# RuyiLian/CheckerPose

Measured on AMD Instinct MI355X. Metric: crops/sec forward (256x256, npt=512), higher is better.
Workload: dtype bf16; 1 GPU; LMO 'ape' hr18GNN2_res6_gnn3Skip_mlpQuery npt=512, PoseNet_GNNskip forward, deterministic random-init weights; global_batch=256, parallelism=dp1 (no forward collective), launch=hipGraph replay of 104 kernel launches

## Files before the change

checkerpose_amd/csrc/common.h:

```cpp
#pragma once
#include <hip/hip_runtime.h>
#include <stdint.h>
#include <atomic>

#include "../../include/checkerpose_hip.h"

typedef __attribute__((ext_vector_type(4))) float f32x4;
typedef __attribute__((ext_vector_type(4))) uint32_t u32x4;
typedef __attribute__((ext_vector_type(2))) uint32_t u32x2;
typedef __attribute__((ext_vector_type(8))) __bf16 bf16x8;

__device__ __forceinline__ float bf16_bits_to_f32(uint32_t h) { return __uint_as_float(h << 16); }
__device__ __forceinline__ uint32_t f32_to_bf16_bits(float f) {
  __bf16 b = (__bf16)f;
  return (uint32_t)__builtin_bit_cast(uint16_t, b);
}
typedef __bf16 cp_bf16x2 __attribute__((ext_vector_type(2)));
typedef float cp_f32x2 __attribute__((ext_vector_type(2)));
__device__ __forceinline__ uint32_t pack_bf16x2(float lo, float hi) {
  return __builtin_bit_cast(uint32_t, __builtin_convertvector(cp_f32x2{lo, hi}, cp_bf16x2));
}

__device__ __forceinline__ float cp_act_slope(int act, float slope) { return act == 1 ? 0.f : (act == 2 ? slope : 1.f); }
__device__ __forceinline__ float cp_act_apply(float v, float s) { return fmaxf(v, fmaf(v, s, 0.f)); }

__device__ __forceinline__ __amdgpu_buffer_rsrc_t cp_dma_rsrc(const void* base) {
  return __builtin_amdgcn_make_buffer_rsrc(const_cast<void*>(base), 0, 0x7fffffff, 0x00020000);
}
__device__ __forceinline__ void cp_lds_dma16(__amdgpu_buffer_rsrc_t rs, uint32_t off, void* lds_dst) {
  __builtin_amdgcn_raw_ptr_buffer_load_lds(rs, (__attribute__((address_space(3))) void*)lds_dst, 16, off, 0, 0, 0);
}

typedef short cp_s16x2 __attribute__((ext_vector_type(2)));
__device__ __forceinline__ uint32_t relu_bf16x2(uint32_t v) {
  return __builtin_bit_cast(uint32_t, __builtin_elementwise_max(__builtin_bit_cast(cp_s16x2, v), cp_s16x2{0, 0}));
}

typedef _Float16 cp_h2 __attribute__((ext_vector_type(2)));
__device__ __forceinline__ uint32_t pack_f16x2_sat(float a, float b) {
  cp_h2 r;
  r.x = (_Float16)__builtin_amdgcn_fmed3f(a, -65504.f, 65504.f);
  r.y = (_Float16)__builtin_amdgcn_fmed3f(b, -65504.f, 65504.f);
  return __builtin_bit_cast(uint32_t, r);
}
__device__ __forceinline__ uint32_t pkmax3_f16(uint32_t a, uint32_t b, uint32_t c) {
  return __builtin_bit_cast(uint32_t, __builtin_elementwise_maximum(__builtin_bit_cast(cp_h2, a),
                            __builtin_elementwise_maximum(__builtin_bit_cast(cp_h2, b), __builtin_bit_cast(cp_h2, c))));
}
__device__ __forceinline__ void pkmax5x4_f16(uint32_t* m, const u32x4& a, const u32x4& b, const u32x4& c, const u32x4& d) {
  asm("v_pk_maximum3_f16 %0, %0, %4, %8\n\t"
      "v_pk_maximum3_f16 %1, %1, %5, %9\n\t"
      "v_pk_maximum3_f16 %2, %2, %6, %10\n\t"
      "v_pk_maximum3_f16 %3, %3, %7, %11\n\t"
      "v_pk_maximum3_f16 %0, %0, %12, %16\n\t"
      "v_pk_maximum3_f16 %1, %1, %13, %17\n\t"
      "v_pk_maximum3_f16 %2, %2, %14, %18\n\t"
      "v_pk_maximum3_f16 %3, %3, %15, %19"
      : "+v"(m[0]), "+v"(m[1]), "+v"(m[2]), "+v"(m[3])
      : "v"(a.x), "v"(a.y), "v"(a.z), "v"(a.w), "v"(b.x), "v"(b.y), "v"(b.z), "v"(b.w),
        "v"(c.x), "v"(c.y), "v"(c.z), "v"(c.w), "v"(d.x), "v"(d.y), "v"(d.z), "v"(d.w));
}
__device__ __forceinline__ float f16_lo(uint32_t w) { return (float)__builtin_bit_cast(cp_h2, w).x; }
__device__ __forceinline__ float f16_hi(uint32_t w) { return (float)__builtin_bit_cast(cp_h2, w).y; }
constexpr uint32_t CP_F16X2_NEG_INF = 0xFC00FC00u;

typedef _Float16 f16x8 __attribute__((ext_vector_type(8)));
template <bool H>
__device__ __forceinline__ f32x4 cp_mma16(const u32x4& w, const u32x4& a, const f32x4& acc) {
  if constexpr (H) return __builtin_amdgcn_mfma_f32_16x16x32_f16(__builtin_bit_cast(f16x8, w), __builtin_bit_cast(f16x8, a), acc, 0, 0, 0);
  else return __builtin_amdgcn_mfma_f32_16x16x32_bf16(__builtin_bit_cast(bf16x8, w), __builtin_bit_cast(bf16x8, a), acc, 0, 0, 0);
}
__device__ __forceinline__ void cp_f16_saturate_on() { asm volatile("s_setreg_imm32_b32 hwreg(HW_REG_MODE, 23, 1), 1" ::: "memory"); }
__device__ __forceinline__ uint32_t pack_f16x2_ovfl(float a, float b) {
  cp_h2 r;
  r.x = (_Float16)a;
  r.y = (_Float16)b;
  return __builtin_bit_cast(uint32_t, r);
}
template <bool H>
__device__ __forceinline__ uint32_t cp_pack2(float lo, float hi) {
  if constexpr (H) return pack_f16x2_ovfl(lo, hi);
  else return pack_bf16x2(lo, hi);
}
template <bool H>
__device__ __forceinline__ u32x4 cp_pack8(const float* f) {
  u32x4 v; v.x = cp_pack2<H>(f[0], f[1]); v.y = cp_pack2<H>(f[2], f[3]); v.z = cp_pack2<H>(f[4], f[5]); v.w = cp_pack2<H>(f[6], f[7]);
  return v;
}
__device__ __forceinline__ uint32_t f32_to_f16_bits_sat(float f) {
  return (uint32_t)__builtin_bit_cast(uint16_t, (_Float16)__builtin_amdgcn_fmed3f(f, -65504.f, 65504.f));
}
__device__ __forceinline__ float f16_bits_to_f32(uint32_t h) { return (float)__builtin_bit_cast(_Float16, (uint16_t)h); }
__device__ __forceinline__ uint32_t f32_to_half_bits(float f, int dtype) { return dtype == CP_F16 ? f32_to_f16_bits_sat(f) : f32_to_bf16_bits(f); }

struct F32Tag { using elem = float; static constexpr int E = 4; static constexpr int dtype = CP_F32; };
struct BF16Tag { using elem = uint16_t; static constexpr int E = 8; static constexpr int dtype = CP_BF16; };
struct F16Tag { using elem = uint16_t; static constexpr int E = 8; static constexpr int dtype = CP_F16; };

template <typename Tag> struct Vec16;
template <> struct Vec16<F32Tag> {
  static __device__ __forceinline__ void unpack(const u32x4& v, float* f) {
    f[0] = __uint_as_float(v.x); f[1] = __uint_as_float(v.y); f[2] = __uint_as_float(v.z); f[3] = __uint_as_float(v.w);
  }
  static __device__ __forceinline__ u32x4 pack(const float* f) {
    u32x4 v; v.x = __float_as_uint(f[0]); v.y = __float_as_uint(f[1]); v.z = __float_as_uint(f[2]); v.w = __float_as_uint(f[3]);
    return v;
  }
};
template <> struct Vec16<BF16Tag> {
  static __device__ __forceinline__ void unpack(const u32x4& v, float* f) {
    f[0] = __uint_as_float(v.x << 16); f[1] = __uint_as_float(v.x & 0xffff0000u);
    f[2] = __uint_as_float(v.y << 16); f[3] = __uint_as_float(v.y & 0xffff0000u);
    f[4] = __uint_as_float(v.z << 16); f[5] = __uint_as_float(v.z & 0xffff0000u);
    f[6] = __uint_as_float(v.w << 16); f[7] = __uint_as_float(v.w & 0xffff0000u);
  }
  static __device__ __forceinline__ u32x4 pack(const float* f) {
    u32x4 v; v.x = pack_bf16x2(f[0], f[1]); v.y = pack_bf16x2(f[2], f[3]);
    v.z = pack_bf16x2(f[4], f[5]); v.w = pack_bf16x2(f[6], f[7]);
    return v;
  }
};

template <> struct Vec16<F16Tag> {
  static __device__ __forceinline__ void unpack(const u32x4& v, float* f) {
    f[0] = f16_lo(v.x); f[1] = f16_hi(v.x); f[2] = f16_lo(v.y); f[3] = f16_hi(v.y);
    f[4] = f16_lo(v.z); f[5] = f16_hi(v.z); f[6] = f16_lo(v.w); f[7] = f16_hi(v.w);
  }
  static __device__ __forceinline__ u32x4 pack(const float* f) { return cp_pack8<true>(f); }
};

__device__ __forceinline__ void cp_up_coord(float s, int o, int n, int& i0, int& step, float& l1) {
#pragma clang fp contract(off)
  const float f = s * (float)o;
  i0 = (int)f;
  step = i0 < n - 1 ? 1 : 0;
  l1 = f - (float)i0;
}
__device__ __forceinline__ float cp_one_minus(float l1) {
#pragma clang fp contract(off)
  return 1.f - l1;
}
__device__ __forceinline__ float cp_bilerp(float a, float b, float c, float d, float lx0, float lx1, float ly0, float ly1) {
#pragma clang fp contract(off)
  const float t = __builtin_fmaf(lx1, b, lx0 * a);
  const float u = __builtin_fmaf(lx1, d, lx0 * c);
  return __builtin_fmaf(ly1, u, ly0 * t);
}

template <typename Tag> __device__ __forceinline__ float load_elem(const void* p, size_t i);
template <> __device__ __forceinline__ float load_elem<F32Tag>(const void* p, size_t i) { return ((const float*)p)[i]; }
template <> __device__ __forceinline__ float load_elem<BF16Tag>(const void* p, size_t i) {
  return bf16_bits_to_f32(((const uint16_t*)p)[i]);
}
template <> __device__ __forceinline__ float load_elem<F16Tag>(const void* p, size_t i) { return f16_bits_to_f32(((const uint16_t*)p)[i]); }
template <typename Tag> __device__ __forceinline__ void store_elem(void* p, size_t i, float v);
template <> __device__ __forceinline__ void store_elem<F16Tag>(void* p, size_t i, float v) { ((uint16_t*)p)[i] = (uint16_t)f32_to_f16_bits_sat(v); }
template <> __device__ __forceinline__ void store_elem<F32Tag>(void* p, size_t i, float v) { ((float*)p)[i] = v; }
template <> __device__ __forceinline__ void store_elem<BF16Tag>(void* p, size_t i, float v) {
  ((uint16_t*)p)[i] = (uint16_t)f32_to_bf16_bits(v);
}

#ifdef CP_DEBUG_KNOBS
#include <stdlib.h>
static inline const char* cp_knob(const char* name) { return getenv(name); }
#else
static inline const char* cp_knob(const char*) { return nullptr; }
#endif
extern std::atomic<int> g_cp_deterministic;
static inline bool cp_deterministic() { return g_cp_deterministic.load(std::memory_order_relaxed) != 0; }
uint32_t* cp_status_word(bool create);
void cp_mark_kernel(const char* fmt, ...);
#define CP_LAUNCH(kernel, ...) do { cp_mark_kernel("%s", #kernel); hipLaunchKernelGGL(kernel, __VA_ARGS__); } while (0)
static inline int cp_check_launch() {
  hipError_t e = hipGetLastError();
  return e == hipSuccess ? CP_OK : CP_ERR_HIP;
}
struct CpDeviceOnce {
  std::atomic<unsigned long long> bits[4];
  bool needed(int dev) const { return !((bits[(dev >> 6) & 3].load(std::memory_order_acquire) >> (dev & 63)) & 1ull); }
  void mark(int dev) { bits[(dev >> 6) & 3].fetch_or(1ull << (dev & 63), std::memory_order_release); }
};
static inline int cp_current_device() {
  int dev = 0;
  return hipGetDevice(&dev) == hipSuccess ? dev : -1;
}
#define CP_LDS_ATTR_ONCE(once, dev, ...)                                                     \
  do {                                                                                       \
    if ((dev) < 0) return CP_ERR_HIP;                                                        \
    if ((once).needed(dev)) {                                                                \
      if (!(__VA_ARGS__)) return CP_ERR_HIP;                                                 \
      (once).mark(dev);                                                                      \
    }                                                                                        \
  } while (0)
static inline bool cp_set_max_lds(const void* fn, size_t bytes) {
  return hipFuncSetAttribute(fn, hipFuncAttributeMaxDynamicSharedMemorySize, (int)bytes) == hipSuccess;
}
static inline int cp_num_cus() {
  static std::atomic<int> cache[256];
  const int dev = cp_current_device();
  if (dev < 0) return 0;
  int n = cache[dev & 255].load(std::memory_order_relaxed);
  if (!n) {
    if (hipDeviceGetAttribute(&n, hipDeviceAttributeMultiprocessorCount, dev) != hipSuccess) return 0;
    cache[dev & 255].store(n, std::memory_order_relaxed);
  }
  return n;
}
static inline bool cp_aligned16(const void* p) { return (((uintptr_t)p) & 15u) == 0; }
static inline size_t cp_align16_up(size_t n) { return (n + 15) & ~(size_t)15; }
static inline bool cp_misaligned(const void* q, uintptr_t mask) { return ((uintptr_t)q & mask) != 0; }
static inline bool cp_act_ok(int act, float slope) { return act != 2  || (slope >= 0.f && slope <= 1.f); }
static inline int cp_elem_size(int dtype) { return (dtype == CP_BF16 || dtype == CP_F16) ? 2 : 4; }
```

checkerpose_amd/csrc/conv3x3_halo.hip:

```cpp
#include <stdlib.h>

#include "common.h"
#include <cstring>

struct HaloParams {
  const void* in; const void* w; const float* scale; const float* shift; const void* res; void* out;
  int B, H, W, Cin, in_cs, in_coff, nchunk, Cout, ngroups, NB;
  int tiles_x, tiles_y, total_tiles;
  int act; float slope;
  uint32_t in_bytes, w_bytes;
  long long o_base, o_sb, o_sy, o_sx;
  int Hs, Ws; float up_sy, up_sx;
  const float* seg_w; const float* seg_b; float* seg_out; int seg_S;
};

constexpr int HTH = 8, HTW = 16, HPW = HTW + 2, HPH = HTH + 2, HNPIX = 192;
constexpr int HPLANE = HNPIX * 16, HBUF = 4 * HPLANE;
constexpr int USRH = 7, USRW = 11, USPIX = 80, USBUF = USPIX * 64;

template <typename Tag> struct MmaH;
template <> struct MmaH<F32Tag> {
  static __device__ __forceinline__ void run(const u32x4& w, const u32x4& a, f32x4& acc) {
    acc = __builtin_amdgcn_mfma_f32_16x16x4f32(__uint_as_float(w.x), __uint_as_float(a.x), acc, 0, 0, 0);
    acc = __builtin_amdgcn_mfma_f32_16x16x4f32(__uint_as_float(w.y), __uint_as_float(a.y), acc, 0, 0, 0);
    acc = __builtin_amdgcn_mfma_f32_16x16x4f32(__uint_as_float(w.z), __uint_as_float(a.z), acc, 0, 0, 0);
    acc = __builtin_amdgcn_mfma_f32_16x16x4f32(__uint_as_float(w.w), __uint_as_float(a.w), acc, 0, 0, 0);
  }
};
template <> struct MmaH<BF16Tag> {
  static __device__ __forceinline__ void run(const u32x4& w, const u32x4& a, f32x4& acc) {
    acc = __builtin_amdgcn_mfma_f32_16x16x32_bf16(__builtin_bit_cast(bf16x8, w), __builtin_bit_cast(bf16x8, a), acc, 0, 0, 0);
  }
};

template <typename Tag, bool HAS_RES>
__global__ __launch_bounds__(256) void conv3x3_halo_kernel(const HaloParams p) {
  constexpr int E = Tag::E;
  constexpr int KCH = 4 * E;
  constexpr int ES = 16 / E;
  extern __shared__ __attribute__((aligned(16))) unsigned char smem[];

  const int label = blockIdx.x & 7, slot = blockIdx.x >> 3;
  const int nblk = slot % p.NB;
  const int t = label * ((p.total_tiles + 7) >> 3) + slot / p.NB;
  if (t >= p.total_tiles) return;
  const int tpi = p.tiles_x * p.tiles_y;
  const int b = t / tpi;
  const int trem = t - b * tpi;
  const int ty = trem / p.tiles_x, tx = trem - ty * p.tiles_x;
  const int y0 = ty * HTH, x0 = tx * HTW;

  const int tid = threadIdx.x;
  const int lane = tid & 63;
  const int wave = __builtin_amdgcn_readfirstlane(tid >> 6);
  const int x = lane & 15, q = lane >> 4;
  const int g = nblk * 4 + wave;
  const bool wave_active = g < p.ngroups;

  const __amdgpu_buffer_rsrc_t rsrc = __builtin_amdgcn_make_buffer_rsrc(const_cast<void*>(p.in), 0, p.in_bytes, 0x00020000);
  const __amdgpu_buffer_rsrc_t wrsrc = __builtin_amdgcn_make_buffer_rsrc(const_cast<void*>(p.w), 0, p.w_bytes, 0x00020000);

  uint32_t s_goff[3];
  uint32_t s_lds[3];
  int s_cq[3];
#pragma unroll
  for (int k = 0; k < 3; ++k) {
    const int i = tid + 256 * k;
    const int hp = i >> 2, pq = i & 3;
    const int py = hp / HPW, px = hp - py * HPW;
    const int gy = y0 - 1 + py, gx = x0 - 1 + px;
    const bool ok = (hp < HPH * HPW) & ((unsigned)gy < (unsigned)p.H) & ((unsigned)gx < (unsigned)p.W);
    s_goff[k] = ok ? (uint32_t)(((b * p.H + gy) * p.W + gx) * p.in_cs + p.in_coff + pq * E) : 0xFFFFFFFFu;
    s_lds[k] = (uint32_t)(pq * HPLANE + (hp < HNPIX ? hp : 0) * 16);
    s_cq[k] = pq * E;
  }
  const bool s_do[3] = {true, true, (tid + 512) < HNPIX * 4};

  auto stage_load = [&](u32x4* v, int c) {
    const int c0 = c * KCH;
#pragma unroll
    for (int k = 0; k < 3; ++k) {
      const bool ok = (s_goff[k] != 0xFFFFFFFFu) & (c0 + s_cq[k] < p.Cin);
      const uint32_t off = ok ? (s_goff[k] + (uint32_t)c0) * ES : 0x80000000u;
      v[k] = __builtin_bit_cast(u32x4, __builtin_amdgcn_raw_buffer_load_b128(rsrc, off, 0, 0));
    }
  };
  auto stage_write = [&](const u32x4* v, int buf) {
#pragma unroll
    for (int k = 0; k < 3; ++k)
      if (s_do[k]) *(u32x4*)(smem + buf * HBUF + s_lds[k]) = v[k];
  };

  f32x4 acc[HTH][2];
#pragma unroll
  for (int mt = 0; mt < HTH; ++mt) { acc[mt][0] = f32x4{0.f, 0.f, 0.f, 0.f}; acc[mt][1] = f32x4{0.f, 0.f, 0.f, 0.f}; }

  const uint32_t wbase = ((uint32_t)(wave_active ? g : 0) * p.nchunk * 18u * 64u + lane) * 16u;
  auto w_load = [&](u32x4* w, int c, int tap) {
    const uint32_t off = wbase + ((uint32_t)c * 18u + (uint32_t)tap * 2u) * 1024u;
    w[0] = __builtin_bit_cast(u32x4, __builtin_amdgcn_raw_buffer_load_b128(wrsrc, off, 0, 0));
    w[1] = __builtin_bit_cast(u32x4, __builtin_amdgcn_raw_buffer_load_b128(wrsrc, off + 1024u, 0, 0));
  };
  const uint32_t a_lane = (uint32_t)(q * HPLANE + x * 16);
  auto a_load = [&](u32x4* a, int buf, int tap) {
    const int r = tap / 3, s = tap - 3 * r;
    const unsigned char* base = smem + buf * HBUF + a_lane + (r * HPW + s) * 16;
#pragma unroll
    for (int mt = 0; mt < HTH; ++mt) a[mt] = *(const u32x4*)(base + mt * HPW * 16);
  };
  auto mma = [&](const u32x4* a, const u32x4* w) {
#pragma unroll
    for (int mt = 0; mt < HTH; ++mt) {
      MmaH<Tag>::run(w[0], a[mt], acc[mt][0]);
      MmaH<Tag>::run(w[1], a[mt], acc[mt][1]);
    }
  };

  u32x4 sv[3];
  stage_load(sv, 0);
  u32x4 w0[2], w1[2], w2[2], aA[HTH], aB[HTH];
  w_load(w0, 0, 0);
  w_load(w1, 0, 1);
  stage_write(sv, 0);
  __syncthreads();

#define CP_TAP(T, ACUR, ANEXT, WCUR, WNEXT, CN, TN)                      \
  w_load(WNEXT, CN, TN);                                                 \
  if (T < 8) a_load(ANEXT, buf, T + 1);                                  \
  __builtin_amdgcn_sched_barrier(0);                                     \
  mma(ACUR, WCUR);                                                       \
  __builtin_amdgcn_sched_barrier(0);
  for (int c = 0; c < p.nchunk; ++c) {
    const int buf = c & 1;
    stage_load(sv, c + 1);
    a_load(aA, buf, 0);
    CP_TAP(0, aA, aB, w0, w2, c, 2)
    CP_TAP(1, aB, aA, w1, w0, c, 3)
    CP_TAP(2, aA, aB, w2, w1, c, 4)
    CP_TAP(3, aB, aA, w0, w2, c, 5)
    CP_TAP(4, aA, aB, w1, w0, c, 6)
    CP_TAP(5, aB, aA, w2, w1, c, 7)
    CP_TAP(6, aA, aB, w0, w2, c, 8)
    CP_TAP(7, aB, aA, w1, w0, c + 1, 0)
    CP_TAP(8, aA, aB, w2, w1, c + 1, 1)
    stage_write(sv, buf ^ 1);
    __syncthreads();
  }
#undef CP_TAP

  if (!wave_active) return;
  const int ch = g * 32 + q * 8;
  if (ch >= p.Cout) return;
  const bool hi_ok = ch + 4 < p.Cout;
  const int ox = x0 + x;
  float sc[8], sh[8];
  {
    const f32x4 s0 = *(const f32x4*)(p.scale + ch), t0 = *(const f32x4*)(p.shift + ch);
    const f32x4 s1 = *(const f32x4*)(p.scale + ch + 4), t1 = *(const f32x4*)(p.shift + ch + 4);
#pragma unroll
    for (int j = 0; j < 4; ++j) { sc[j] = s0[j]; sh[j] = t0[j]; sc[4 + j] = s1[j]; sh[4 + j] = t1[j]; }
  }
  if (ox >= p.W) return;
  float rvv[HAS_RES ? HTH : 1][8];
  if constexpr (HAS_RES) {
#pragma unroll
    for (int mt = 0; mt < HTH; ++mt) {
      const int oy = y0 + mt;
#pragma unroll
      for (int j = 0; j < 8; ++j) rvv[mt][j] = 0.f;
      if (oy >= p.H) continue;
      const long long o = p.o_base + (long long)b * p.o_sb + (long long)oy * p.o_sy + (long long)ox * p.o_sx + ch;
      if (E == 4) {
        const f32x4 r0 = *(const f32x4*)((const float*)p.res + o);
#pragma unroll
        for (int j = 0; j < 4; ++j) rvv[mt][j] = r0[j];
        if (hi_ok) {
          const f32x4 r1 = *(const f32x4*)((const float*)p.res + o + 4);
#pragma unroll
          for (int j = 0; j < 4; ++j) rvv[mt][4 + j] = r1[j];
        }
      } else {
        const u32x2 r0 = *(const u32x2*)((const uint16_t*)p.res + o);
        rvv[mt][0] = __uint_as_float(r0.x << 16); rvv[mt][1] = __uint_as_float(r0.x & 0xffff0000u);
        rvv[mt][2] = __uint_as_float(r0.y << 16); rvv[mt][3] = __uint_as_float(r0.y & 0xffff0000u);
        if (hi_ok) {
          const u32x2 r1 = *(const u32x2*)((const uint16_t*)p.res + o + 4);
          rvv[mt][4] = __uint_as_float(r1.x << 16); rvv[mt][5] = __uint_as_float(r1.x & 0xffff0000u);
          rvv[mt][6] = __uint_as_float(r1.y << 16); rvv[mt][7] = __uint_as_float(r1.y & 0xffff0000u);
        }
      }
    }
  }
#pragma unroll
  for (int mt = 0; mt < HTH; ++mt) {
    const int oy = y0 + mt;
    if (oy >= p.H) continue;
    const long long o = p.o_base + (long long)b * p.o_sb + (long long)oy * p.o_sy + (long long)ox * p.o_sx + ch;
    float v[8];
#pragma unroll
    for (int j = 0; j < 4; ++j) { v[j] = acc[mt][0][j] * sc[j] + sh[j]; v[4 + j] = acc[mt][1][j] * sc[4 + j] + sh[4 + j]; }
    if constexpr (HAS_RES) {
#pragma unroll
      for (int j = 0; j < 8; ++j) v[j] += rvv[HAS_RES ? mt : 0][j];
    }
#pragma unroll
    for (int j = 0; j < 8; ++j) {
      v[j] = cp_act_apply(v[j], cp_act_slope(p.act, p.slope));
    }
    if (E == 4) {
      *(f32x4*)((float*)p.out + o) = f32x4{v[0], v[1], v[2], v[3]};
      if (hi_ok) *(f32x4*)((float*)p.out + o + 4) = f32x4{v[4], v[5], v[6], v[7]};
    } else {
      if (hi_ok) {
        u32x4 pk; pk.x = pack_bf16x2(v[0], v[1]); pk.y = pack_bf16x2(v[2], v[3]); pk.z = pack_bf16x2(v[4], v[5]); pk.w = pack_bf16x2(v[6], v[7]);
        if ((((uintptr_t)((uint16_t*)p.out + o)) & 15u) == 0) *(u32x4*)((uint16_t*)p.out + o) = pk;
        else { *(u32x2*)((uint16_t*)p.out + o) = u32x2{pk.x, pk.y}; *(u32x2*)((uint16_t*)p.out + o + 4) = u32x2{pk.z, pk.w}; }
      } else {
        u32x2 pk; pk.x = pack_bf16x2(v[0], v[1]); pk.y = pack_bf16x2(v[2], v[3]);
        *(u32x2*)((uint16_t*)p.out + o) = pk;
      }
    }
  }
}


template <typename Tag, bool HAS_RES, bool UP = false, bool SEG = false>
__global__ __launch_bounds__(256, 2) void conv3x3_halo4_kernel(const HaloParams p) {
  constexpr int E = Tag::E;
  constexpr int KCH = 4 * E;
  constexpr int ES = 16 / E;
  extern __shared__ __attribute__((aligned(16))) unsigned char smem[];
  unsigned char* const sSrc = smem + 2 * HBUF;

  const int label = blockIdx.x & 7, slot = blockIdx.x >> 3;
  const int nblk = slot % p.NB;
  const int t = label * ((p.total_tiles + 7) >> 3) + slot / p.NB;
  if (t >= p.total_tiles) return;
  const int tpi = p.tiles_x * p.tiles_y;
  const int b = t / tpi;
  const int trem = t - b * tpi;
  const int ty = trem / p.tiles_x, tx = trem - ty * p.tiles_x;
  const int y0 = ty * HTH, x0 = tx * HTW;

  const int tid = threadIdx.x;
  const int lane = tid & 63;
  const int wave = __builtin_amdgcn_readfirstlane(tid >> 6);
  const int x = lane & 15, q = lane >> 4;
  const int g = nblk * 4 + wave;

  const __amdgpu_buffer_rsrc_t rsrc = __builtin_amdgcn_make_buffer_rsrc(const_cast<void*>(p.in), 0, p.in_bytes, 0x00020000);
  const __amdgpu_buffer_rsrc_t wrsrc = __builtin_amdgcn_make_buffer_rsrc(const_cast<void*>(p.w), 0, p.w_bytes, 0x00020000);

  uint32_t s_goff[3], s_lds[3];
  int s_cq[3];
#pragma unroll
  for (int k = 0; k < 3; ++k) {
    const int i = tid + 256 * k;
    const int hp = i >> 2, pq = i & 3;
    const int py = hp / HPW, px = hp - py * HPW;
    const int gy = y0 - 1 + py, gx = x0 - 1 + px;
    const bool ok = (hp < HPH * HPW) & ((unsigned)gy < (unsigned)p.H) & ((unsigned)gx < (unsigned)p.W);
    s_goff[k] = ok ? (uint32_t)(((b * p.H + gy) * p.W + gx) * p.in_cs + p.in_coff + pq * E) : 0xFFFFFFFFu;
    s_lds[k] = (uint32_t)(pq * HPLANE + hp * 16);
    s_cq[k] = pq * E;
  }
  auto stage_load = [&](u32x4* v, int c) {
    const int c0 = c * KCH;
#pragma unroll
    for (int k = 0; k < 3; ++k) {
      const bool ok = (s_goff[k] != 0xFFFFFFFFu) & (c0 + s_cq[k] < p.Cin);
      v[k] = __builtin_bit_cast(u32x4, __builtin_amdgcn_raw_buffer_load_b128(rsrc, ok ? (s_goff[k] + (uint32_t)c0) * ES : 0x80000000u, 0, 0));
    }
  };
  auto stage_write = [&](const u32x4* v, int buf) {
#pragma unroll
    for (int k = 0; k < 3; ++k) *(u32x4*)(smem + buf * HBUF + s_lds[k]) = v[k];
  };

  uint32_t u_goff[2], m_off[3];
  float m_lx[3], m_ly[3];
  if constexpr (UP) {
    int sy0, sx0, st_; float fr_;
    cp_up_coord(p.up_sy, y0 > 0 ? y0 - 1 : 0, p.Hs, sy0, st_, fr_);
    cp_up_coord(p.up_sx, x0 > 0 ? x0 - 1 : 0, p.Ws, sx0, st_, fr_);
#pragma unroll
    for (int k = 0; k < 2; ++k) {
      const int i = tid + 256 * k;
      const int sp = i >> 2, pq = i & 3;
      const int ry = sp / USRW, rx = sp - ry * USRW;
      const int yy = sy0 + ry, xx = sx0 + rx;
      const bool ok = (sp < USRH * USRW) & (yy < p.Hs) & (xx < p.Ws);
      u_goff[k] = ok ? (uint32_t)(((b * p.Hs + yy) * p.Ws + xx) * p.in_cs + p.in_coff + pq * E) : 0xFFFFFFFFu;
    }
#pragma unroll
    for (int k = 0; k < 3; ++k) {
      const int i = tid + 256 * k;
      const int hp = i >> 2, pq = i & 3;
      const int py = hp / HPW, px = hp - py * HPW;
      const int gy = y0 - 1 + py, gx = x0 - 1 + px;
      const bool ok = (hp < HPH * HPW) & ((unsigned)gy < (unsigned)p.H) & ((unsigned)gx < (unsigned)p.W);
      int iy0, ix0, my, mx;
      cp_up_coord(p.up_sy, gy, p.Hs, iy0, my, m_ly[k]);
      cp_up_coord(p.up_sx, gx, p.Ws, ix0, mx, m_lx[k]);
      m_off[k] = ok ? (uint32_t)((((iy0 - sy0) * USRW + (ix0 - sx0)) * 4 + pq) * 16) | (uint32_t)(mx | (my << 1) | 4) : 0u;
    }
  }
  auto src_load = [&](u32x4* v, int c) {
    const int c0 = c * KCH;
#pragma unroll
    for (int k = 0; k < 2; ++k) {
      const bool ok = (u_goff[k] != 0xFFFFFFFFu) & (c0 + (tid & 3) * E < p.Cin);
      v[k] = __builtin_bit_cast(u32x4, __builtin_amdgcn_raw_buffer_load_b128(rsrc, ok ? (u_goff[k] + (uint32_t)c0) * ES : 0x80000000u, 0, 0));
    }
  };
  auto src_write = [&](const u32x4* v, int sb) {
    *(u32x4*)(sSrc + sb * USBUF + tid * 16) = v[0];
    if (tid < USPIX * 4 - 256) *(u32x4*)(sSrc + sb * USBUF + (tid + 256) * 16) = v[1];
  };
  auto interp = [&](int k, int sb, int hb) {
    const uint32_t mo = m_off[k];
    const unsigned char* s00 = sSrc + sb * USBUF + (mo & ~15u);
    const uint32_t dx = (mo & 1u) ? 64u : 0u, dy = (mo & 2u) ? (uint32_t)(USRW * 64) : 0u;
    const float lx1 = m_lx[k], lx0 = cp_one_minus(lx1), ly1 = m_ly[k], ly0 = cp_one_minus(ly1);
    const bool in_img = (mo & 4u) != 0u;
    unsigned char* dst = smem + hb * HBUF + s_lds[k];
#pragma unroll
    for (int j = 0; j < 4; ++j) {
      const uint32_t r00 = *(const uint32_t*)(s00 + 4 * j), r01 = *(const uint32_t*)(s00 + dx + 4 * j);
      const uint32_t r10 = *(const uint32_t*)(s00 + dy + 4 * j), r11 = *(const uint32_t*)(s00 + dy + dx + 4 * j);
      uint32_t o;
      if constexpr (E == 4) {
        o = __float_as_uint(cp_bilerp(__uint_as_float(r00), __uint_as_float(r01), __uint_as_float(r10), __uint_as_float(r11), lx0, lx1, ly0, ly1));
      } else {
        const float lo = cp_bilerp(__uint_as_float(r00 << 16), __uint_as_float(r01 << 16), __uint_as_float(r10 << 16), __uint_as_float(r11 << 16), lx0, lx1, ly0, ly1);
        const float hi = cp_bilerp(__uint_as_float(r00 & 0xffff0000u), __uint_as_float(r01 & 0xffff0000u), __uint_as_float(r10 & 0xffff0000u),
                                   __uint_as_float(r11 & 0xffff0000u), lx0, lx1, ly0, ly1);
        o = pack_bf16x2(lo, hi);
      }
      *(uint32_t*)(dst + 4 * j) = in_img ? o : 0u;
    }
  };

  f32x4 acc[HTH][4];
#pragma unroll
  for (int mt = 0; mt < HTH; ++mt)
#pragma unroll
    for (int nt = 0; nt < 4; ++nt) acc[mt][nt] = f32x4{0.f, 0.f, 0.f, 0.f};

  const uint32_t wbase = ((uint32_t)g * p.nchunk * 36u * 64u + lane) * 16u;
  auto w_load = [&](u32x4* w, int c, int tap) {
    const uint32_t off = wbase + ((uint32_t)c * 36u + (uint32_t)tap * 4u) * 1024u;
#pragma unroll
    for (int nt = 0; nt < 4; ++nt) w[nt] = __builtin_bit_cast(u32x4, __builtin_amdgcn_raw_buffer_load_b128(wrsrc, off + nt * 1024u, 0, 0));
  };
  const uint32_t a_lane = (uint32_t)(q * HPLANE + x * 16);
  auto a_load = [&](u32x4* a, int buf, int tap, int half) {
    const int r = tap / 3, s2 = tap - 3 * r;
    const unsigned char* base = smem + buf * HBUF + a_lane + ((r + 4 * half) * HPW + s2) * 16;
#pragma unroll
    for (int i = 0; i < 4; ++i) a[i] = *(const u32x4*)(base + i * HPW * 16);
  };
  auto mma = [&](const u32x4* a, const u32x4* w, int half) {
#pragma unroll
    for (int i = 0; i < 4; ++i)
#pragma unroll
      for (int nt = 0; nt < 4; ++nt) MmaH<Tag>::run(w[nt], a[i], acc[4 * half + i][nt]);
  };

  u32x4 sv[3];
  u32x4 wA[4], wB[4], a0[4], a1[4];
  if constexpr (UP) {
    src_load(sv, 0);
    w_load(wA, 0, 0);
    src_write(sv, 0);
    src_load(sv, 1);
    __syncthreads();
    interp(0, 0, 0); interp(1, 0, 0); interp(2, 0, 0);
    src_write(sv, 1);
  } else {
    stage_load(sv, 0);
    w_load(wA, 0, 0);
    stage_write(sv, 0);
  }
  __syncthreads();

#define CP_TAP4(T, WCUR, WNEXT, CN, TN)                                                 \
  a_load(a1, buf, T, 1); w_load(WNEXT, CN, TN); __builtin_amdgcn_sched_barrier(0);       \
  mma(a0, WCUR, 0); __builtin_amdgcn_sched_barrier(0);                                   \
  if (T < 8) a_load(a0, buf, T + 1, 0);                                                  \
  __builtin_amdgcn_sched_barrier(0);                                                     \
  mma(a1, WCUR, 1); __builtin_amdgcn_sched_barrier(0);
  for (int c = 0; c < p.nchunk; ++c) {
    const int buf = c & 1;
    if constexpr (UP) src_load(sv, c + 2); else stage_load(sv, c + 1);
    a_load(a0, buf, 0, 0);
    CP_TAP4(0, wA, wB, c, 1)
    CP_TAP4(1, wB, wA, c, 2)
    if constexpr (UP) { __builtin_amdgcn_sched_barrier(0); interp(0, buf ^ 1, buf ^ 1); __builtin_amdgcn_sched_barrier(0); }
    CP_TAP4(2, wA, wB, c, 3)
    CP_TAP4(3, wB, wA, c, 4)
    CP_TAP4(4, wA, wB, c, 5)
    if constexpr (UP) { __builtin_amdgcn_sched_barrier(0); interp(1, buf ^ 1, buf ^ 1); __builtin_amdgcn_sched_barrier(0); }
    CP_TAP4(5, wB, wA, c, 6)
    CP_TAP4(6, wA, wB, c, 7)
    CP_TAP4(7, wB, wA, c, 8)
    if constexpr (UP) { __builtin_amdgcn_sched_barrier(0); interp(2, buf ^ 1, buf ^ 1); __builtin_amdgcn_sched_barrier(0); }
    CP_TAP4(8, wA, wB, c + 1, 0)
#pragma unroll
    for (int nt = 0; nt < 4; ++nt) wA[nt] = wB[nt];
    if constexpr (UP) src_write(sv, buf); else stage_write(sv, buf ^ 1);
    __syncthreads();
  }
#undef CP_TAP4

  const int ch = g * 64 + q * 16;
  const int ox = x0 + x;
  if constexpr (!SEG) { if (ox >= p.W) return; }
  const bool xok = SEG ? ox < p.W : true;
  constexpr int SMAX = 2;
  float segw[SEG ? SMAX : 1][16], segp[SEG ? 8 : 1][SEG ? SMAX : 1];
  if constexpr (SEG) {
#pragma unroll
    for (int s_ = 0; s_ < SMAX; ++s_) {
#pragma unroll
      for (int k = 0; k < 4; ++k) {
        const f32x4 w4 = s_ < p.seg_S ? *(const f32x4*)(p.seg_w + (size_t)s_ * p.Cout + ch + 4 * k) : f32x4{0.f, 0.f, 0.f, 0.f};
#pragma unroll
        for (int j = 0; j < 4; ++j) segw[s_][4 * k + j] = w4[j];
      }
#pragma unroll
      for (int mt = 0; mt < 8; ++mt) segp[mt][s_] = 0.f;
    }
  }
  float sc[16], sh[16];
#pragma unroll
  for (int nt = 0; nt < 4; ++nt) {
    const f32x4 s4 = *(const f32x4*)(p.scale + ch + 4 * nt), t4 = *(const f32x4*)(p.shift + ch + 4 * nt);
#pragma unroll
    for (int j = 0; j < 4; ++j) { sc[4 * nt + j] = s4[j]; sh[4 * nt + j] = t4[j]; }
  }
#pragma unroll
  for (int half = 0; half < 2; ++half) {
    u32x4 rr[HAS_RES ? 4 : 1][E == 4 ? 4 : 2];
    if constexpr (HAS_RES) {
#pragma unroll
      for (int i = 0; i < 4; ++i) {
        const int oy = y0 + 4 * half + i;
        const long long o = p.o_base + (long long)b * p.o_sb + (long long)oy * p.o_sy + (long long)ox * p.o_sx + ch;
#pragma unroll
        for (int k = 0; k < (E == 4 ? 4 : 2); ++k) {
          rr[i][k] = u32x4{0u, 0u, 0u, 0u};
          if (oy < p.H) rr[i][k] = E == 4 ? *(const u32x4*)((const float*)p.res + o + 4 * k) : *(const u32x4*)((const uint16_t*)p.res + o + 8 * k);
        }
      }
    }
#pragma unroll
    for (int i = 0; i < 4; ++i) {
      const int mt = 4 * half + i;
      const int oy = y0 + mt;
      if (oy >= p.H) continue;
      const long long o = p.o_base + (long long)b * p.o_sb + (long long)oy * p.o_sy + (long long)ox * p.o_sx + ch;
      float v[16];
#pragma unroll
      for (int nt = 0; nt < 4; ++nt)
#pragma unroll
        for (int j = 0; j < 4; ++j) v[4 * nt + j] = acc[mt][nt][j] * sc[4 * nt + j] + sh[4 * nt + j];
      if constexpr (HAS_RES) {
        if (E == 4) {
#pragma unroll
          for (int k = 0; k < 4; ++k) {
            v[4 * k + 0] += __uint_as_float(rr[i][k].x); v[4 * k + 1] += __uint_as_float(rr[i][k].y);
            v[4 * k + 2] += __uint_as_float(rr[i][k].z); v[4 * k + 3] += __uint_as_float(rr[i][k].w);
          }
        } else {
          float r8[8];
#pragma unroll
          for (int k = 0; k < 2; ++k) {
            Vec16<BF16Tag>::unpack(rr[i][k], r8);
#pragma unroll
            for (int j = 0; j < 8; ++j) v[8 * k + j] += r8[j];
          }
        }
      }
#pragma unroll
      for (int j = 0; j < 16; ++j) {
        v[j] = cp_act_apply(v[j], cp_act_slope(p.act, p.slope));
      }
      if (E == 4) {
        if (xok) {
#pragma unroll
          for (int k = 0; k < 4; ++k) *(f32x4*)((float*)p.out + o + 4 * k) = f32x4{v[4 * k], v[4 * k + 1], v[4 * k + 2], v[4 * k + 3]};
        }
      } else {
        const u32x4 pk0 = Vec16<BF16Tag>::pack(v), pk1 = Vec16<BF16Tag>::pack(v + 8);
        if (xok) {
          *(u32x4*)((uint16_t*)p.out + o) = pk0;
          *(u32x4*)((uint16_t*)p.out + o + 8) = pk1;
        }
        if constexpr (SEG) { Vec16<BF16Tag>::unpack(pk0, v); Vec16<BF16Tag>::unpack(pk1, v + 8); }
      }
      if constexpr (SEG) {
#pragma unroll
        for (int s_ = 0; s_ < SMAX; ++s_) {
          float a = 0.f;
#pragma unroll
          for (int j = 0; j < 16; ++j) a += v[j] * segw[s_][j];
          segp[mt][s_] = a;
        }
      }
    }
  }
  if constexpr (SEG) {
    float* const red = (float*)smem;
#pragma unroll
    for (int mt = 0; mt < 8; ++mt)
#pragma unroll
      for (int s_ = 0; s_ < SMAX; ++s_) {
        float a = segp[mt][s_];
        a += __shfl_xor(a, 16);
        a += __shfl_xor(a, 32);
        if (q == 0) red[((wave * 8 + mt) * 16 + x) * SMAX + s_] = a;
      }
    __syncthreads();
    const int s_ = tid & 1, px = tid >> 1;
    const int mt = px >> 4, xx = px & 15;
    const int oy = y0 + mt, oxx = x0 + xx;
    if (s_ < p.seg_S && oy < p.H && oxx < p.W) {
      float a = p.seg_b[s_];
#pragma unroll
      for (int wv = 0; wv < 4; ++wv) a += red[((wv * 8 + mt) * 16 + xx) * SMAX + s_];
      p.seg_out[(((size_t)b * p.seg_S + s_) * p.H + oy) * p.W + oxx] = a;
    }
  }
}

template <typename Tag>
__global__ void pack_halo4_weight_kernel(const float* __restrict__ w, void* __restrict__ out, int Cout, int Cin, int nchunk,
                                         size_t total) {
  constexpr int E = Tag::E;
  const size_t i = (size_t)blockIdx.x * blockDim.x + threadIdx.x;
  if (i >= total) return;
  const int e = (int)(i % E);
  const int lane = (int)((i / E) % 64);
  size_t blk = i / (E * 64);
  const int nt = (int)(blk % 4); blk /= 4;
  const int tap = (int)(blk % 9); blk /= 9;
  const int c = (int)(blk % nchunk);
  const int g = (int)(blk / nchunk);
  const int row = lane & 15, kq = lane >> 4;
  const int n = g * 64 + (row >> 2) * 16 + nt * 4 + (row & 3);
  const int cin = c * (4 * E) + kq * E + e;
  float v = 0.f;
  if (n < Cout && cin < Cin) v = w[((size_t)n * Cin + cin) * 9 + tap];
  store_elem<Tag>(out, i, v);
}

static inline bool halo_wide(int Cout) { return Cout >= 256 && Cout % 256 == 0 && !cp_knob("CP_NO_HALO4"); }

template <typename Tag, int NT, int KS = 3>
__global__ __launch_bounds__(256) void conv3x3_halo_s_kernel(const HaloParams p) {
  if (KS == 2 && p.seg_S == CP_F16) cp_f16_saturate_on();
  constexpr int E = Tag::E;
  constexpr int KCH = 4 * E;
  constexpr int ES = 16 / E;
  constexpr int NTAP = KS * KS;
  constexpr int WPIECES = NTAP * NT * 64;
  constexpr int WITER = (WPIECES + 255) / 256;
  extern __shared__ __attribute__((aligned(16))) unsigned char smem[];
  unsigned char* const sA = smem;
  unsigned char* const sW = smem + HBUF;

  const int t = blockIdx.x;
  const int tpi = p.tiles_x * p.tiles_y;
  const int b = t / tpi;
  const int trem = t - b * tpi;
  const int ty = trem / p.tiles_x, tx = trem - ty * p.tiles_x;
  const int y0 = ty * HTH, x0 = tx * HTW;

  const int tid = threadIdx.x;
  const int lane = tid & 63;
  const int wave = __builtin_amdgcn_readfirstlane(tid >> 6);
  const int x = lane & 15, q = lane >> 4;

  const __amdgpu_buffer_rsrc_t rsrc = __builtin_amdgcn_make_buffer_rsrc(const_cast<void*>(p.in), 0, p.in_bytes, 0x00020000);
  const __amdgpu_buffer_rsrc_t wrsrc = __builtin_amdgcn_make_buffer_rsrc(const_cast<void*>(p.w), 0, p.w_bytes, 0x00020000);

  uint32_t s_goff[3], s_lds[3];
  int s_cq[3];
#pragma unroll
  for (int k = 0; k < 3; ++k) {
    const int i = tid + 256 * k;
    const int hp = i >> 2, pq = i & 3;
    const int py = hp / HPW, px = hp - py * HPW;
    const int gy = y0 - 1 + py, gx = x0 - 1 + px;
    const bool ok = (hp < HPH * HPW) & ((unsigned)gy < (unsigned)p.H) & ((unsigned)gx < (unsigned)p.W);
    s_goff[k] = ok ? (uint32_t)(((b * p.H + gy) * p.W + gx) * p.in_cs + p.in_coff + pq * E) : 0xFFFFFFFFu;
    s_lds[k] = (uint32_t)(pq * HPLANE + hp * 16);
    s_cq[k] = pq * E;
  }

  f32x4 acc[2][NT];
#pragma unroll
  for (int mt = 0; mt < 2; ++mt)
#pragma unroll
    for (int nt = 0; nt < NT; ++nt) acc[mt][nt] = f32x4{0.f, 0.f, 0.f, 0.f};

  const uint32_t a_lane = (uint32_t)(q * HPLANE + (2 * wave * HPW + x) * 16);
  const int OH = p.H + (3 - KS), OW = p.W + (3 - KS);
  const int ox = x0 + x;
  const int chq = q * 4 * NT;
  long long obase[2];
  bool rok[2];
#pragma unroll
  for (int mt = 0; mt < 2; ++mt) {
    const int oy = y0 + 2 * wave + mt;
    rok[mt] = (oy < OH) & (ox < OW);
    obase[mt] = p.o_base + (long long)b * p.o_sb + (long long)oy * p.o_sy + (long long)ox * p.o_sx + chq;
  }
  f32x4 rv[2][NT];
  if (p.res) {
#pragma unroll
    for (int mt = 0; mt < 2; ++mt)
#pragma unroll
      for (int nt = 0; nt < NT; ++nt) {
        rv[mt][nt] = f32x4{0.f, 0.f, 0.f, 0.f};
        if (rok[mt] && chq + nt * 4 < p.Cout) {
          if (E == 4) rv[mt][nt] = *(const f32x4*)((const float*)p.res + obase[mt] + nt * 4);
          else {
            const u32x2 r2 = *(const u32x2*)((const uint16_t*)p.res + obase[mt] + nt * 4);
            rv[mt][nt] = f32x4{__uint_as_float(r2.x << 16), __uint_as_float(r2.x & 0xffff0000u),
                               __uint_as_float(r2.y << 16), __uint_as_float(r2.y & 0xffff0000u)};
          }
        }
      }
  }
  for (int c = 0; c < p.nchunk; ++c) {
    const int c0 = c * KCH;
    u32x4 sv[3], wv[WITER];
#pragma unroll
    for (int k = 0; k < 3; ++k) {
      const bool ok = (s_goff[k] != 0xFFFFFFFFu) & (c0 + s_cq[k] < p.Cin);
      const uint32_t off = ok ? (s_goff[k] + (uint32_t)c0) * ES : 0x80000000u;
      sv[k] = __builtin_bit_cast(u32x4, __builtin_amdgcn_raw_buffer_load_b128(rsrc, off, 0, 0));
    }
#pragma unroll
    for (int k = 0; k < WITER; ++k) {
      const int i = tid + 256 * k;
      const uint32_t off = i < WPIECES ? ((uint32_t)c * WPIECES + (uint32_t)i) * 16u : 0x80000000u;
      wv[k] = __builtin_bit_cast(u32x4, __builtin_amdgcn_raw_buffer_load_b128(wrsrc, off, 0, 0));
    }
    if (c > 0) __syncthreads();
#pragma unroll
    for (int k = 0; k < 3; ++k) *(u32x4*)(sA + s_lds[k]) = sv[k];
#pragma unroll
    for (int k = 0; k < WITER; ++k) {
      const int i = tid + 256 * k;
      if (i < WPIECES) *(u32x4*)(sW + i * 16) = wv[k];
    }
    __syncthreads();
#pragma unroll
    for (int tap = 0; tap < NTAP; ++tap) {
      const int r = tap / KS, s2 = tap - KS * r;
      const unsigned char* ab = sA + a_lane + (r * HPW + s2) * 16;
      const u32x4 a0 = *(const u32x4*)(ab);
      const u32x4 a1 = *(const u32x4*)(ab + HPW * 16);
#pragma unroll
      for (int nt = 0; nt < NT; ++nt) {
        const u32x4 w = *(const u32x4*)(sW + (tap * NT + nt) * 1024 + lane * 16);
        MmaH<Tag>::run(w, a0, acc[0][nt]);
        MmaH<Tag>::run(w, a1, acc[1][nt]);
      }
    }
  }

  if (ox >= OW) return;
#pragma unroll
  for (int mt = 0; mt < 2; ++mt) {
    if (!rok[mt]) continue;
#pragma unroll
    for (int nt = 0; nt < NT; ++nt) {
      const int ch = chq + nt * 4;
      if (ch >= p.Cout) continue;
      const f32x4 sc = *(const f32x4*)(p.scale + ch), sh = *(const f32x4*)(p.shift + ch);
      float v[4];
#pragma unroll
      for (int j = 0; j < 4; ++j) v[j] = acc[mt][nt][j] * sc[j] + sh[j];
      if (p.res) {
#pragma unroll
        for (int j = 0; j < 4; ++j) v[j] += rv[mt][nt][j];
      }
#pragma unroll
      for (int j = 0; j < 4; ++j) {
        v[j] = cp_act_apply(v[j], cp_act_slope(p.act, p.slope));
      }
      if (E == 4) *(f32x4*)((float*)p.out + obase[mt] + nt * 4) = f32x4{v[0], v[1], v[2], v[3]};
      else if (KS == 2 && p.seg_S == CP_F16) {
        u32x2 pk; pk.x = cp_pack2<true>(v[0], v[1]); pk.y = cp_pack2<true>(v[2], v[3]); *(u32x2*)((uint16_t*)p.out + obase[mt] + nt * 4) = pk;
      }
      else { u32x2 pk; pk.x = pack_bf16x2(v[0], v[1]); pk.y = pack_bf16x2(v[2], v[3]); *(u32x2*)((uint16_t*)p.out + obase[mt] + nt * 4) = pk; }
    }
  }
}

constexpr int FXW = HTW + 4, FXH = HTH + 4, FXPLANE = 256 * 16;

template <typename Tag, int NT>
__global__ __launch_bounds__(256) void basicblock_fused_kernel(const HaloParams p, const void* __restrict__ w2,
                                                               const float* __restrict__ scale2, const float* __restrict__ shift2) {
  constexpr int E = Tag::E;
// ... 721 lines not shown
```

Measured before the change: 24380 crops/s.

## Interleave bilinear upsample micro-steps between MFMA instructions in halo conv

```diff
diff --git a/checkerpose_amd/csrc/common.h b/checkerpose_amd/csrc/common.h
--- a/checkerpose_amd/csrc/common.h
+++ b/checkerpose_amd/csrc/common.h
@@ -146,6 +146,11 @@
   const float u = __builtin_fmaf(lx1, d, lx0 * c);
   return __builtin_fmaf(ly1, u, ly0 * t);
 }
+__device__ __forceinline__ float cp_lerp_mul(float l0, float a) {
+#pragma clang fp contract(off)
+  return l0 * a;
+}
+__device__ __forceinline__ float cp_lerp_fma(float l1, float b, float t) { return __builtin_fmaf(l1, b, t); }
 
 template <typename Tag> __device__ __forceinline__ float load_elem(const void* p, size_t i);
 template <> __device__ __forceinline__ float load_elem<F32Tag>(const void* p, size_t i) { return ((const float*)p)[i]; }
diff --git a/checkerpose_amd/csrc/conv3x3_halo.hip b/checkerpose_amd/csrc/conv3x3_halo.hip
--- a/checkerpose_amd/csrc/conv3x3_halo.hip
+++ b/checkerpose_amd/csrc/conv3x3_halo.hip
@@ -16,7 +16,7 @@
 
 constexpr int HTH = 8, HTW = 16, HPW = HTW + 2, HPH = HTH + 2, HNPIX = 192;
 constexpr int HPLANE = HNPIX * 16, HBUF = 4 * HPLANE;
-constexpr int USRH = 7, USRW = 11, USPIX = 80, USBUF = USPIX * 64;
+constexpr int USRH = 7, USRW = 11, USPIX = 80, USQ = 82 * 8, USPL = 2 * USQ, USBUF = 4 * USPL;
 
 template <typename Tag> struct MmaH;
 template <> struct MmaH<F32Tag> {
@@ -277,8 +277,9 @@
     for (int k = 0; k < 3; ++k) *(u32x4*)(smem + buf * HBUF + s_lds[k]) = v[k];
   };
 
-  uint32_t u_goff[2], m_off[3];
-  float m_lx[3], m_ly[3];
+  uint32_t u_goff[2], m_src[3];
+  float m_lx0[3], m_lx1[3], m_ly0[3], m_ly1[3];
+  bool m_in[3];
   if constexpr (UP) {
     int sy0, sx0, st_; float fr_;
     cp_up_coord(p.up_sy, y0 > 0 ? y0 - 1 : 0, p.Hs, sy0, st_, fr_);
@@ -288,9 +289,8 @@
       const int i = tid + 256 * k;
       const int sp = i >> 2, pq = i & 3;
       const int ry = sp / USRW, rx = sp - ry * USRW;
-      const int yy = sy0 + ry, xx = sx0 + rx;
-      const bool ok = (sp < USRH * USRW) & (yy < p.Hs) & (xx < p.Ws);
-      u_goff[k] = ok ? (uint32_t)(((b * p.Hs + yy) * p.Ws + xx) * p.in_cs + p.in_coff + pq * E) : 0xFFFFFFFFu;
+      const int yy = min(sy0 + ry, p.Hs - 1), xx = min(sx0 + rx, p.Ws - 1);
+      u_goff[k] = sp < USRH * USRW ? (uint32_t)(((b * p.Hs + yy) * p.Ws + xx) * p.in_cs + p.in_coff + pq * E) : 0xFFFFFFFFu;
     }
 #pragma unroll
     for (int k = 0; k < 3; ++k) {
@@ -300,9 +300,12 @@
       const int gy = y0 - 1 + py, gx = x0 - 1 + px;
       const bool ok = (hp < HPH * HPW) & ((unsigned)gy < (unsigned)p.H) & ((unsigned)gx < (unsigned)p.W);
       int iy0, ix0, my, mx;
-      cp_up_coord(p.up_sy, gy, p.Hs, iy0, my, m_ly[k]);
-      cp_up_coord(p.up_sx, gx, p.Ws, ix0, mx, m_lx[k]);
-      m_off[k] = ok ? (uint32_t)((((iy0 - sy0) * USRW + (ix0 - sx0)) * 4 + pq) * 16) | (uint32_t)(mx | (my << 1) | 4) : 0u;
+      cp_up_coord(p.up_sy, gy, p.Hs, iy0, my, m_ly1[k]);
+      cp_up_coord(p.up_sx, gx, p.Ws, ix0, mx, m_lx1[k]);
+      m_ly0[k] = cp_one_minus(m_ly1[k]);
+      m_lx0[k] = cp_one_minus(m_lx1[k]);
+      m_in[k] = ok;
+      m_src[k] = (uint32_t)(2 * HBUF + pq * USPL + (ok ? ((iy0 - sy0) * USRW + (ix0 - sx0)) * 8 : 0));
     }
   }
   auto src_load = [&](u32x4* v, int c) {
@@ -314,32 +317,59 @@
     }
   };
   auto src_write = [&](const u32x4* v, int sb) {
-    *(u32x4*)(sSrc + sb * USBUF + tid * 16) = v[0];
-    if (tid < USPIX * 4 - 256) *(u32x4*)(sSrc + sb * USBUF + (tid + 256) * 16) = v[1];
-  };
-  auto interp = [&](int k, int sb, int hb) {
-    const uint32_t mo = m_off[k];
-    const unsigned char* s00 = sSrc + sb * USBUF + (mo & ~15u);
-    const uint32_t dx = (mo & 1u) ? 64u : 0u, dy = (mo & 2u) ? (uint32_t)(USRW * 64) : 0u;
-    const float lx1 = m_lx[k], lx0 = cp_one_minus(lx1), ly1 = m_ly[k], ly0 = cp_one_minus(ly1);
-    const bool in_img = (mo & 4u) != 0u;
-    unsigned char* dst = smem + hb * HBUF + s_lds[k];
-#pragma unroll
-    for (int j = 0; j < 4; ++j) {
-      const uint32_t r00 = *(const uint32_t*)(s00 + 4 * j), r01 = *(const uint32_t*)(s00 + dx + 4 * j);
-      const uint32_t r10 = *(const uint32_t*)(s00 + dy + 4 * j), r11 = *(const uint32_t*)(s00 + dy + dx + 4 * j);
-      uint32_t o;
-      if constexpr (E == 4) {
-        o = __float_as_uint(cp_bilerp(__uint_as_float(r00), __uint_as_float(r01), __uint_as_float(r10), __uint_as_float(r11), lx0, lx1, ly0, ly1));
-      } else {
-        const float lo = cp_bilerp(__uint_as_float(r00 << 16), __uint_as_float(r01 << 16), __uint_as_float(r10 << 16), __uint_as_float(r11 << 16), lx0, lx1, ly0, ly1);
-        const float hi = cp_bilerp(__uint_as_float(r00 & 0xffff0000u), __uint_as_float(r01 & 0xffff0000u), __uint_as_float(r10 & 0xffff0000u),
-                                   __uint_as_float(r11 & 0xffff0000u), lx0, lx1, ly0, ly1);
-        o = pack_bf16x2(lo, hi);
-      }
-      *(uint32_t*)(dst + 4 * j) = in_img ? o : 0u;
-    }
-  };
+    unsigned char* d = sSrc + sb * USBUF + (tid & 3) * USPL + (tid >> 2) * 8;
+    *(u32x2*)(d) = u32x2{v[0].x, v[0].y};
+    *(u32x2*)(d + USQ) = u32x2{v[0].z, v[0].w};
+    if (tid < USPIX * 4 - 256) {
+      *(u32x2*)(d + 64 * 8) = u32x2{v[1].x, v[1].y};
+      *(u32x2*)(d + 64 * 8 + USQ) = u32x2{v[1].z, v[1].w};
+    }
+  };
+  u32x2 ur[4];
+  uint32_t uo[2];
+  float ua[2], ub[2], ut[2], uu[2];
+  constexpr int NV = E == 4 ? 1 : 2;
+#define CP_UP_FENCE(V) asm("" : "+v"(V))
+  auto up_unpack = [&](uint32_t r, float* v) {
+    if constexpr (E == 4) v[0] = __uint_as_float(r);
+    else { v[0] = __uint_as_float(r << 16); v[1] = __uint_as_float(r & 0xffff0000u); CP_UP_FENCE(v[1]); }
+  };
+  auto lx0 = [&](int k) { return E == 4 ? cp_one_minus(m_lx1[k]) : m_lx0[k]; };
+  auto ly0 = [&](int k) { return E == 4 ? cp_one_minus(m_ly1[k]) : m_ly0[k]; };
+  auto up_micro = [&](int gi, int m, int sb, int hb) {
+    const int hs = gi / 3, ph = gi - 3 * hs, k = hs >> 1, h = hs & 1, j = ph - 1;
+    if (ph == 0) {
+      if (m == 0) {
+        const u32x2* s00 = (const u32x2*)(smem + sb * USBUF + m_src[k]);
+        ur[0] = s00[h * (USQ / 8)];
+        ur[1] = s00[h * (USQ / 8) + 1];
+        ur[2] = s00[h * (USQ / 8) + USRW];
+        ur[3] = s00[h * (USQ / 8) + USRW + 1];
+      }
+      return;
+    }
+    switch (m) {
+      case 0: up_unpack(ur[0][j], ua); break;
+      case 1: up_unpack(ur[1][j], ub); break;
+      case 2: for (int e = 0; e < NV; ++e) { ut[e] = cp_lerp_mul(lx0(k), ua[e]); if (e) CP_UP_FENCE(ut[e]); } break;
+      case 3: for (int e = 0; e < NV; ++e) { ut[e] = cp_lerp_fma(m_lx1[k], ub[e], ut[e]); if (e) CP_UP_FENCE(ut[e]); } break;
+      case 4: up_unpack(ur[2][j], ua); break;
+      case 5: up_unpack(ur[3][j], ub); break;
+      case 6: for (int e = 0; e < NV; ++e) { uu[e] = cp_lerp_mul(lx0(k), ua[e]); if (e) CP_UP_FENCE(uu[e]); } break;
+      case 7: for (int e = 0; e < NV; ++e) { uu[e] = cp_lerp_fma(m_lx1[k], ub[e], uu[e]); if (e) CP_UP_FENCE(uu[e]); } break;
+      case 8: for (int e = 0; e < NV; ++e) { ut[e] = cp_lerp_mul(ly0(k), ut[e]); if (e) CP_UP_FENCE(ut[e]); } break;
+      case 9: for (int e = 0; e < NV; ++e) { ut[e] = cp_lerp_fma(m_ly1[k], uu[e], ut[e]); if (e) CP_UP_FENCE(ut[e]); } break;
+      case 10: {
+        uint32_t o;
+        if constexpr (E == 4) o = __float_as_uint(ut[0]); else o = pack_bf16x2(ut[0], ut[1]);
+        uo[j] = m_in[k] ? o : 0u;
+        if constexpr (E == 4) ((uint32_t*)(smem + hb * HBUF + s_lds[0]))[256 * k + 2 * h + j] = uo[j];
+      } break;
+      case 11: if (E != 4 && ph == 2) ((u32x2*)(smem + hb * HBUF + s_lds[0]))[128 * k + h] = u32x2{uo[0], uo[1]}; break;
+      default: break;
+    }
+  };
+#undef CP_UP_FENCE
 
   f32x4 acc[HTH][4];
 #pragma unroll
@@ -365,6 +395,17 @@
     for (int i = 0; i < 4; ++i)
 #pragma unroll
       for (int nt = 0; nt < 4; ++nt) MmaH<Tag>::run(w[nt], a[i], acc[4 * half + i][nt]);
+  };
+  auto mma_up = [&](const u32x4* a, const u32x4* w, int half, int gi, int sb, int hb) {
+#pragma unroll
+    for (int i = 0; i < 4; ++i)
+#pragma unroll
+      for (int nt = 0; nt < 4; ++nt) {
+        MmaH<Tag>::run(w[nt], a[i], acc[4 * half + i][nt]);
+        __builtin_amdgcn_sched_barrier(0);
+        up_micro(gi, 4 * i + nt, sb, hb);
+        __builtin_amdgcn_sched_barrier(0);
+      }
   };
 
   u32x4 sv[3];
@@ -375,7 +416,10 @@
     src_write(sv, 0);
     src_load(sv, 1);
     __syncthreads();
-    interp(0, 0, 0); interp(1, 0, 0); interp(2, 0, 0);
+#pragma unroll
+    for (int gi = 0; gi < 18; ++gi)
+#pragma unroll
+      for (int m = 0; m < 12; ++m) up_micro(gi, m, 0, 0);
     src_write(sv, 1);
   } else {
     stage_load(sv, 0);
@@ -386,25 +430,26 @@
 
 #define CP_TAP4(T, WCUR, WNEXT, CN, TN)                                                 \
   a_load(a1, buf, T, 1); w_load(WNEXT, CN, TN); __builtin_amdgcn_sched_barrier(0);       \
-  mma(a0, WCUR, 0); __builtin_amdgcn_sched_barrier(0);                                   \
+  if constexpr (UP) mma_up(a0, WCUR, 0, 2 * T, buf ^ 1, buf ^ 1);    \
+  else mma(a0, WCUR, 0);                                                                 \
+  __builtin_amdgcn_sched_barrier(0);                                                     \
   if (T < 8) a_load(a0, buf, T + 1, 0);                                                  \
   __builtin_amdgcn_sched_barrier(0);                                                     \
-  mma(a1, WCUR, 1); __builtin_amdgcn_sched_barrier(0);
+  if constexpr (UP) mma_up(a1, WCUR, 1, 2 * T + 1, buf ^ 1, buf ^ 1);                    \
+  else mma(a1, WCUR, 1);                                                                 \
+  __builtin_amdgcn_sched_barrier(0);
   for (int c = 0; c < p.nchunk; ++c) {
     const int buf = c & 1;
     if constexpr (UP) src_load(sv, c + 2); else stage_load(sv, c + 1);
     a_load(a0, buf, 0, 0);
     CP_TAP4(0, wA, wB, c, 1)
     CP_TAP4(1, wB, wA, c, 2)
-    if constexpr (UP) { __builtin_amdgcn_sched_barrier(0); interp(0, buf ^ 1, buf ^ 1); __builtin_amdgcn_sched_barrier(0); }
     CP_TAP4(2, wA, wB, c, 3)
     CP_TAP4(3, wB, wA, c, 4)
     CP_TAP4(4, wA, wB, c, 5)
-    if constexpr (UP) { __builtin_amdgcn_sched_barrier(0); interp(1, buf ^ 1, buf ^ 1); __builtin_amdgcn_sched_barrier(0); }
     CP_TAP4(5, wB, wA, c, 6)
     CP_TAP4(6, wA, wB, c, 7)
     CP_TAP4(7, wB, wA, c, 8)
-    if constexpr (UP) { __builtin_amdgcn_sched_barrier(0); interp(2, buf ^ 1, buf ^ 1); __builtin_amdgcn_sched_barrier(0); }
     CP_TAP4(8, wA, wB, c + 1, 0)
 #pragma unroll
     for (int nt = 0; nt < 4; ++nt) wA[nt] = wB[nt];
```

Result: faster. 24920 crops/s (median of 6 runs) (+2.2%).
